# showlab/VideoSwap

Measured on NVIDIA H100. Metric: denoise-steps/sec, 16f 512^2 SD1.5 UNet3D (CFG UNet fwd + CFG combine + DDIM step), higher is better.
Workload: dtype f16

## Files before the change

videoswap_b200/csrc/attention.cu:

```cuda
#include "common.cuh"
#include "kernels.h"

namespace vs {
namespace {

__device__ __forceinline__ void cp_async16(uint32_t dst, const void* src, bool pred) {
  const int sz = pred ? 16 : 0;
  asm volatile("cp.async.cg.shared.global [%0], [%1], 16, %2;" ::"r"(dst), "l"(src), "r"(sz) : "memory");
}
__device__ __forceinline__ void cp_async_commit() { asm volatile("cp.async.commit_group;" ::: "memory"); }
template <int N>
__device__ __forceinline__ void cp_async_wait() {
  asm volatile("cp.async.wait_group %0;" ::"n"(N) : "memory");
}
__device__ __forceinline__ void ldsm_x4(uint32_t addr, uint32_t& r0, uint32_t& r1, uint32_t& r2, uint32_t& r3) {
  asm volatile("ldmatrix.sync.aligned.m8n8.x4.shared.b16 {%0,%1,%2,%3}, [%4];"
               : "=r"(r0), "=r"(r1), "=r"(r2), "=r"(r3)
               : "r"(addr));
}
__device__ __forceinline__ void ldsm_x4_t(uint32_t addr, uint32_t& r0, uint32_t& r1, uint32_t& r2, uint32_t& r3) {
  asm volatile("ldmatrix.sync.aligned.m8n8.x4.trans.shared.b16 {%0,%1,%2,%3}, [%4];"
               : "=r"(r0), "=r"(r1), "=r"(r2), "=r"(r3)
               : "r"(addr));
}
__device__ __forceinline__ void mma16816(float* c, const uint32_t* a, uint32_t b0, uint32_t b1) {
  asm volatile(
      "mma.sync.aligned.m16n8k16.row.col.f32.f16.f16.f32 {%0,%1,%2,%3}, {%4,%5,%6,%7}, {%8,%9}, {%0,%1,%2,%3};"
      : "+f"(c[0]), "+f"(c[1]), "+f"(c[2]), "+f"(c[3])
      : "r"(a[0]), "r"(a[1]), "r"(a[2]), "r"(a[3]), "r"(b0), "r"(b1));
}
__device__ __forceinline__ uint32_t pack_h2(float a, float b) {
  __half2 h = __floats2half2_rn(a, b);
  return *reinterpret_cast<uint32_t*>(&h);
}

template <int DP, int NT>
__device__ __forceinline__ void warp_qk(float (*s)[4], uint32_t q_s, uint32_t k_s, int lds_bytes, int lane) {
#pragma unroll
  for (int n = 0; n < NT; ++n) s[n][0] = s[n][1] = s[n][2] = s[n][3] = 0.f;
#pragma unroll
  for (int kk = 0; kk < DP / 16; ++kk) {
    uint32_t a[4];
    ldsm_x4(q_s + (lane & 15) * lds_bytes + (kk * 16 + (lane >> 4) * 8) * 2, a[0], a[1], a[2], a[3]);
#pragma unroll
    for (int n = 0; n < NT; n += 2) {
      uint32_t b0, b1, b2, b3;
      const int key = n * 8 + (lane & 7) + ((lane >> 4) ? 8 : 0);
// ... 584 lines not shown
```

videoswap_b200/csrc/common.cuh:

```cuda
#pragma once
#include <cuda.h>
#include <cuda_fp16.h>
#include <cuda_runtime.h>
#include <stdint.h>
#include <stdio.h>

namespace vs {

void set_error(const char* fmt, ...);
const char* last_error();

#define VS_CHECK_CUDA(expr)                                                                         \
  do {                                                                                              \
    cudaError_t _e = (expr);                                                                        \
    if (_e != cudaSuccess) {                                                                        \
      vs::set_error("%s:%d CUDA error %s: %s", __FILE__, __LINE__, #expr, cudaGetErrorString(_e)); \
      return 1;                                                                                     \
    }                                                                                               \
  } while (0)

#define VS_REQUIRE(cond, ...)                \
  do {                                       \
    if (!(cond)) {                           \
      vs::set_error(__VA_ARGS__);            \
// ... 100 lines not shown
      ::"r"(dst), "l"(reinterpret_cast<uint64_t>(m)), "r"(bar), "r"(c0), "r"(c1), "r"(c2), "r"(c3)
      : "memory");
}

__device__ __forceinline__ bool elect_one() {
  uint32_t pred;
  asm volatile(
      "{\n\t.reg .pred P;\n\t"
      "elect.sync _|P, 0xffffffff;\n\t"
      "selp.u32 %0, 1, 0, P;\n\t}"
      : "=r"(pred));
  return pred != 0;
}

__device__ __forceinline__ uint32_t cluster_ctarank() {
  uint32_t r;
  asm volatile("mov.u32 %0, %%cluster_ctarank;" : "=r"(r));
  return r;
}
__device__ __forceinline__ void cluster_sync_all() {
  asm volatile("barrier.cluster.arrive.release.aligned;" ::: "memory");
  asm volatile("barrier.cluster.wait.acquire.aligned;" ::: "memory");
}
__device__ __forceinline__ uint32_t mapa_shared(uint32_t addr, uint32_t rank) {
  uint32_t r;
  asm volatile("mapa.shared::cluster.u32 %0, %1, %2;" : "=r"(r) : "r"(addr), "r"(rank));
  return r;
}
__device__ __forceinline__ void named_bar_sync(int id, int nthreads) {
  asm volatile("bar.sync %0, %1;" ::"r"(id), "r"(nthreads) : "memory");
}
__device__ __forceinline__ void named_bar_arrive(int id, int nthreads) {
  asm volatile("bar.arrive %0, %1;" ::"r"(id), "r"(nthreads) : "memory");
}

__device__ __forceinline__ void pdl_trigger() { asm volatile("griddepcontrol.launch_dependents;" ::: "memory"); }
__device__ __forceinline__ void pdl_wait() { asm volatile("griddepcontrol.wait;" ::: "memory"); }

template <int N>
__device__ __forceinline__ void setmaxnreg_dec() { asm volatile("setmaxnreg.dec.sync.aligned.u32 %0;" ::"n"(N)); }
template <int N>
__device__ __forceinline__ void setmaxnreg_inc() { asm volatile("setmaxnreg.inc.sync.aligned.u32 %0;" ::"n"(N)); }

__device__ __forceinline__ void wgmma_fence() { asm volatile("wgmma.fence.sync.aligned;" ::: "memory"); }
__device__ __forceinline__ void wgmma_commit() { asm volatile("wgmma.commit_group.sync.aligned;" ::: "memory"); }
template <int N>
__device__ __forceinline__ void wgmma_wait() { asm volatile("wgmma.wait_group.sync.aligned %0;" ::"n"(N) : "memory"); }

__device__ __forceinline__ uint64_t gmma_desc_sw128(uint32_t smem_addr) {
  uint64_t d = 0;
  d |= (uint64_t)((smem_addr & 0x3FFFF) >> 4);
  d |= (uint64_t)1 << 16;
  d |= (uint64_t)(1024 >> 4) << 32;
  d |= (uint64_t)1 << 62;
  return d;
}
__device__ __forceinline__ uint64_t gmma_desc_sw128_mn(uint32_t smem_addr, uint32_t lbo_bytes) {
  uint64_t d = 0;
  d |= (uint64_t)((smem_addr & 0x3FFFF) >> 4);
  d |= (uint64_t)((lbo_bytes >> 4) & 0x3FFF) << 16;
  d |= (uint64_t)(1024 >> 4) << 32;
  d |= (uint64_t)1 << 62;
  return d;
}

#define VS_R8(i) "+f"(d[i]), "+f"(d[i + 1]), "+f"(d[i + 2]), "+f"(d[i + 3]), "+f"(d[i + 4]), "+f"(d[i + 5]), "+f"(d[i + 6]), "+f"(d[i + 7])
// ... 93 lines not shown
```

videoswap_b200/csrc/gemm.cu:

```cuda
#include <type_traits>

#include "common.cuh"
#include "kernels.h"

namespace vs {

namespace {

constexpr int BM = 128;
constexpr int WG_M = 64;
constexpr int BK = 64;
constexpr int A_STAGE_BYTES = BM * BK * 2;
constexpr uint64_t A_HALF_DESC = (WG_M * BK * 2) >> 4;
constexpr int GEMM_THREADS = 384;
constexpr int SMEM_LIMIT = 227 * 1024;
constexpr int EPI_COLS = 32;
constexpr int EPI_WARP_BYTES = 16 * 64;
constexpr int EPI_BYTES = 8 * EPI_WARP_BYTES;
constexpr int PRODUCER_REGS = 40, CONSUMER_REGS = 232;
enum { EPI_F_GEGLU = 1, EPI_F_RES = 2, EPI_F_RV = 4, EPI_F_LN = 8, EPI_F_LNOUT = 16, EPI_F_QGELU = 32 };

struct GemmParams {
  CUtensorMap tmA, tmA2, tmB;
  int M, N;
  int num_kb;
  int kb_per_tap;
  int kb_src1;
  int taps;
  int a_rank;
  int nimg, H, W, TH, TW, TN, tiles_x, tiles_y;
  int tap_x0, tap_y0, tap_w;
  int osy, osx, ooy, oox, OH, OW;
  int tw_log, thw_log;
  int m_tiles, n_tiles;
  const float* bias;
  const float* rowvec;
  int ldrv;
  int pix_per_batch;
  int rv_mod;
  const float2* ln_stats;
  const float* ln_u;
  const float2* ln_parts;
  int ln_nparts;
  float ln_inv_c;
  float2* ln_sums_out;
  const __half* residual;
  int ldr;
  __half* out;
  int ldc;
  int staged;
  int stages;
};

struct GemmParamsSub : GemmParams {
  CUtensorMap tmS[3];
  int sub_short;
};

struct GemmParamsS2 : GemmParams {
  CUtensorMap tmP[3];
};

template <int BN>
struct Cfg {
  static constexpr bool COOP = BN > 160;
  static constexpr int HALVES = COOP ? 1 : 2;
  static constexpr int B_STAGE_BYTES = BN * BK * 2;
  static constexpr int STAGE_BYTES = A_STAGE_BYTES + B_STAGE_BYTES;
  static constexpr int STAGES_RAW = (SMEM_LIMIT - 2048 - EPI_BYTES) / STAGE_BYTES;
  static constexpr int STAGES = STAGES_RAW > 12 ? 12 : STAGES_RAW;
  static constexpr int SMEM_BYTES = STAGES * STAGE_BYTES + EPI_BYTES + 1024  + 256 ;
  static_assert(B_STAGE_BYTES % 1024 == 0, "B stage must keep 1024-byte alignment for SWIZZLE_128B");
  static_assert(STAGES >= 3, "pipeline too shallow");
  static_assert(BN % 32 == 0 && BN <= 256, "wgmma N");
};

__device__ __forceinline__ uint32_t sw64_off(int row, int chunk) {
  return (uint32_t)(row * 64 + ((chunk ^ ((row >> 1) & 3)) << 4));
}

template <int BN, int EPI, typename Params>
__global__ void __launch_bounds__(GEMM_THREADS, 1) gemm_tc_kernel(const __grid_constant__ Params p) {
  using C = Cfg<BN>;
  constexpr bool SUB = std::is_same<Params, GemmParamsSub>::value;
  constexpr bool S2 = std::is_same<Params, GemmParamsS2>::value;
  constexpr bool GEGLU = (EPI & EPI_F_GEGLU) != 0, HAS_RES = (EPI & EPI_F_RES) != 0, HAS_RV = (EPI & EPI_F_RV) != 0;
  constexpr bool LN = (EPI & EPI_F_LN) != 0;
  constexpr bool LNOUT = (EPI & EPI_F_LNOUT) != 0;
  constexpr bool QGELU = (EPI & EPI_F_QGELU) != 0;
  extern __shared__ uint8_t smem_raw[];
  const uint32_t smem_base = (smem_u32(smem_raw) + 1023u) & ~1023u;
  const uint32_t epi_base = smem_base + C::STAGES * C::STAGE_BYTES;
  const uint32_t bar_base = epi_base + EPI_BYTES;
  auto full_bar = [&](int s) { return bar_base + 8u * s; };
  auto empty_bar = [&](int s) { return bar_base + 8u * (C::STAGES + s); };

  const int warp = threadIdx.x >> 5;
  const int lane = threadIdx.x & 31;
  const int wg = threadIdx.x >> 7;
  const int nst = (p.stages > 0 && p.stages < C::STAGES) ? p.stages : C::STAGES;
  const int total_tiles = p.m_tiles * p.n_tiles;

  if (threadIdx.x == 0) {
    prefetch_tmap(&p.tmA);
    prefetch_tmap(&p.tmB);
    if (p.kb_src1 < p.kb_per_tap) prefetch_tmap(&p.tmA2);
    if constexpr (SUB) {
      if (p.sub_short & 1) prefetch_tmap(&p.tmS[0]);
      if (p.sub_short & 2) prefetch_tmap(&p.tmS[1]);
      if (p.sub_short == 3) prefetch_tmap(&p.tmS[2]);
    }
    if constexpr (S2) {
      for (int k = 0; k < 3; ++k) prefetch_tmap(&p.tmP[k]);
    }
    for (int s = 0; s < C::STAGES; ++s) {
      mbar_init(full_bar(s), 1);
      mbar_init(empty_bar(s), C::COOP ? 8 : 4);
    }
    fence_barrier_init();
  }
  __syncthreads();
  pdl_trigger();
  pdl_wait();

  if (wg == 0) {
    setmaxnreg_dec<PRODUCER_REGS>();
// ... 27 lines not shown
          if constexpr (SUB) {
            const bool sy = short_y && dy == p.tap_y0 + 2, sx = short_x && dx == tap_x0 + 2;
            if (sy || sx) tm = sy ? (sx ? &p.tmS[2] : &p.tmS[0]) : &p.tmS[1];
          }
          int ox = dx, oy = dy;
          if constexpr (S2) {
            const int par = ((dy & 1) << 1) | (dx & 1);
            if (par) tm = &p.tmP[par - 1];
            ox = dx >> 1; oy = dy >> 1;
          }
          const int c = (first ? r : r - kb_src1) * BK;
          mbar_expect_tx(fb, C::STAGE_BYTES);
          if (conv) tma_load_4d(a_dst, tm, fb, c, x0 + ox, y0 + oy, i0);
          else tma_load_2d(a_dst, tm, fb, c, m0);
          tma_load_2d(a_dst + A_STAGE_BYTES, &p.tmB, fb, kcoord, n0);
        }
        __syncwarp();
        kcoord += BK;
        if (++r == kb_per_tap) {
          r = 0;
          if (++dx == tap_x1) { dx = tap_x0; ++dy; }
        }
        if (++pr_s == (uint32_t)nst) { pr_s = 0; pr_ph ^= 1; }
      }
    }
    return;
  }

  setmaxnreg_inc<CONSUMER_REGS>();
  const int g = wg - 1;
  const int wq = warp & 3;
  const int q = lane & 3;
  const int rbase = 16 * wq + (lane >> 2);
  const uint32_t stage_buf = epi_base + (uint32_t)(warp - 4) * EPI_WARP_BYTES;
  const bool has_bias = p.bias != nullptr;
  const bool staged = p.staged != 0;
  const int num_kb = p.num_kb;
  auto tile_pixel = [&](int m_tile, int row) -> int {
    if (p.a_rank == 4) {
      const int x0 = (m_tile % p.tiles_x) * p.TW;
      const int y0 = ((m_tile / p.tiles_x) % p.tiles_y) * p.TH;
      const int i0 = (m_tile / (p.tiles_x * p.tiles_y)) * p.TN;
      const int ti = row >> p.thw_log, rem = row & ((1 << p.thw_log) - 1);
      const int y = y0 + (rem >> p.tw_log), x = x0 + (rem & (p.TW - 1)), img = i0 + ti;
      if constexpr (SUB) {
        const int oy = y * p.osy + p.ooy, ox = x * p.osx + p.oox;
        return ((img < p.nimg) && (y < p.H) && (x < p.W) && (oy < p.OH) && (ox < p.OW)) ? (img * p.OH + oy) * p.OW + ox : -1;
      }
      return ((img < p.nimg) && (y < p.H) && (x < p.W)) ? (img * p.OH + y * p.osy + p.ooy) * p.OW + x * p.osx + p.oox : -1;
    }
    const int px = m_tile * BM + row;
    return px < p.M ? px : -1;
  };

  const int bar_mine = 1 + g, bar_other = 2 - g;
  float acc[C::HALVES][BN / 2];
  uint32_t s = 0, ph = 0;
  for (int t = blockIdx.x, j = 0; t < total_tiles; t += gridDim.x, ++j) {
    const int m_tile = t / p.n_tiles, n_tile = t % p.n_tiles;
    if (!C::COOP && (j & 1) != g) {
      const uint32_t sn = s + (uint32_t)num_kb;
      ph ^= (sn / (uint32_t)nst) & 1u;
      s = sn % (uint32_t)nst;
      continue;
    }
    if (!C::COOP && j > 0) named_bar_sync(bar_mine, 256);
    uint32_t prev = 0;
    for (int kb = 0; kb < num_kb; ++kb) {
      mbar_wait(full_bar(s), ph);
      wgmma_fence();
      const uint32_t a_addr = smem_base + s * C::STAGE_BYTES;
      const uint64_t da = gmma_desc_sw128(a_addr) + (C::COOP ? (uint64_t)g * A_HALF_DESC : 0);
      const uint64_t db = gmma_desc_sw128(a_addr + A_STAGE_BYTES);
#pragma unroll
      for (int k = 0; k < BK / 16; ++k) {
#pragma unroll
        for (int hh = 0; hh < C::HALVES; ++hh)
          wgmma_ss<BN>(acc[hh], da + hh * A_HALF_DESC + 2 * k, db + 2 * k, (kb | k) != 0 ? 1u : 0u);
      }
      wgmma_commit();
      if (kb > 0) {
        wgmma_wait<1>();
        if (lane == 0) mbar_arrive(empty_bar(prev));
      }
      prev = s;
      if (++s == (uint32_t)nst) { s = 0; ph ^= 1; }
    }
    if (!C::COOP && t + (int)gridDim.x < total_tiles) named_bar_arrive(bar_other, 256);
    wgmma_wait<0>();
    if (lane == 0) mbar_arrive(empty_bar(prev));

    const int n0 = n_tile * BN;
#pragma unroll
    for (int hh = 0; hh < C::HALVES; ++hh) {
      const int r0 = WG_M * (C::COOP ? g : hh) + rbase;
      int pix[2];
      pix[0] = tile_pixel(m_tile, r0);
      pix[1] = tile_pixel(m_tile, r0 + 8);
      const float* rv[2] = {nullptr, nullptr};
      if (HAS_RV || !staged) {
#pragma unroll
        for (int h = 0; h < 2; ++h) {
          if (p.rowvec != nullptr && pix[h] >= 0) {
            int ri = pix[h] / p.pix_per_batch;
            if (p.rv_mod > 0) ri %= p.rv_mod;
            rv[h] = p.rowvec + (long long)ri * p.ldrv + n0;
          }
        }
      }
      if (staged) {
        constexpr int OC = GEGLU ? BN / 2 : BN;
        const int oc0 = n_tile * OC;
        const int nsub = (p.N - n0 < BN ? (GEGLU ? (p.N - n0) / 2 : p.N - n0) : OC) / EPI_COLS;
        float la[2] = {1.f, 1.f}, lb[2] = {0.f, 0.f};
        if (LN) {
#pragma unroll
          for (int h = 0; h < 2; ++h) {
            if (pix[h] < 0) continue;
            if (p.ln_nparts > 0) {
              float S = 0.f, Q = 0.f;
              for (int k = 0; k < p.ln_nparts; ++k) {
                const float2 v = __ldg(p.ln_parts + (long long)k * p.M + pix[h]);
                S += v.x; Q += v.y;
              }
              const float mean = S * p.ln_inv_c;
              la[h] = rsqrtf(fmaxf(fmaf(-mean, mean, Q * p.ln_inv_c), 0.f) + 1e-5f);
              lb[h] = -mean * la[h];
            } else {
              const float2 st2 = __ldg(p.ln_stats + pix[h]);
              la[h] = st2.x; lb[h] = st2.y;
            }
          }
        }
        float rs[2] = {0.f, 0.f}, rq[2] = {0.f, 0.f};
        __half* orow[2];
        const __half* rrow[2];
#pragma unroll
        for (int h = 0; h < 2; ++h) {
          const long long px = pix[h] >= 0 ? pix[h] : 0;
          orow[h] = p.out + px * p.ldc + oc0 + q * 8;
          rrow[h] = HAS_RES ? p.residual + px * p.ldr + oc0 + q * 8 : nullptr;
        }
#pragma unroll
        for (int sb = 0; sb < OC / EPI_COLS; ++sb) {
          if (sb >= nsub) break;
          uint4 rr[2];
          if (HAS_RES) {
#pragma unroll
            for (int h = 0; h < 2; ++h) rr[h] = __ldg(reinterpret_cast<const uint4*>(rrow[h] + sb * EPI_COLS));
          }
#pragma unroll
          for (int jj = 0; jj < 4; ++jj) {
            const int j = 4 * sb + jj;
            const int c = 8 * j + 2 * q;
            float2 b = has_bias ? __ldg(reinterpret_cast<const float2*>(p.bias + n0 + c)) : make_float2(0.f, 0.f);
            float2 u = LN ? __ldg(reinterpret_cast<const float2*>(p.ln_u + n0 + c)) : make_float2(0.f, 0.f);
            float2 bg = make_float2(0.f, 0.f), ug = make_float2(0.f, 0.f);
            if (GEGLU) {
              bg = __ldg(reinterpret_cast<const float2*>(p.bias + n0 + BN / 2 + c));
              if (LN) ug = __ldg(reinterpret_cast<const float2*>(p.ln_u + n0 + BN / 2 + c));
            }
#pragma unroll
            for (int h = 0; h < 2; ++h) {
              float f0 = acc[hh][4 * j + 2 * h], f1 = acc[hh][4 * j + 2 * h + 1];
              if (GEGLU) {
                float g0 = acc[hh][4 * (j + BN / 16) + 2 * h], g1 = acc[hh][4 * (j + BN / 16) + 2 * h + 1];
                float bv0 = b.x, bv1 = b.y, bg0 = bg.x, bg1 = bg.y;
                if (LN) {
                  bv0 = fmaf(lb[h], u.x, bv0); bv1 = fmaf(lb[h], u.y, bv1);
                  bg0 = fmaf(lb[h], ug.x, bg0); bg1 = fmaf(lb[h], ug.y, bg1);
                  f0 *= la[h]; f1 *= la[h]; g0 *= la[h]; g1 *= la[h];
                }
                f0 = (f0 + bv0) * gelu_sig(g0 + bg0);
                f1 = (f1 + bv1) * gelu_sig(g1 + bg1);
              } else {
                if (LN) {
                  f0 = fmaf(la[h], f0, fmaf(lb[h], u.x, b.x));
                  f1 = fmaf(la[h], f1, fmaf(lb[h], u.y, b.y));
                } else if (has_bias) {
                  f0 += b.x; f1 += b.y;
                }
                if (HAS_RV && rv[h] != nullptr) {
                  const float2 r2 = __ldg(reinterpret_cast<const float2*>(rv[h] + c));
                  f0 += r2.x; f1 += r2.y;
                }
                if constexpr (QGELU) {
                  f0 = quick_gelu_f(f0); f1 = quick_gelu_f(f1);
                }
              }
              const __half2 hv = __floats2half2_rn(f0, f1);
              asm volatile("st.shared.b32 [%0], %1;" ::"r"(stage_buf + sw64_off((lane >> 2) + 8 * h, jj) + 4 * q),
                           "r"(*reinterpret_cast<const uint32_t*>(&hv)) : "memory");
            }
          }
          __syncwarp();
#pragma unroll
          for (int h = 0; h < 2; ++h) {
            uint4 o;
            asm volatile("ld.shared.v4.b32 {%0,%1,%2,%3}, [%4];" : "=r"(o.x), "=r"(o.y), "=r"(o.z), "=r"(o.w)
                         : "r"(stage_buf + sw64_off((lane >> 2) + 8 * h, q)));
            if (HAS_RES) {
              __half2* oh = reinterpret_cast<__half2*>(&o);
              const __half2* rh = reinterpret_cast<const __half2*>(&rr[h]);
#pragma unroll
              for (int t = 0; t < 4; ++t) oh[t] = __hadd2(oh[t], rh[t]);
            }
            if (pix[h] >= 0) *reinterpret_cast<uint4*>(orow[h] + sb * EPI_COLS) = o;
            if (LNOUT) {
              const __half2* oh = reinterpret_cast<const __half2*>(&o);
              const float2 a = __half22float2(oh[0]), b2 = __half22float2(oh[1]), c2 = __half22float2(oh[2]), d2 = __half22float2(oh[3]);
              rs[h] += ((a.x + a.y) + (b2.x + b2.y)) + ((c2.x + c2.y) + (d2.x + d2.y));
              float q0 = fmaf(a.x, a.x, a.y * a.y), q1 = fmaf(b2.x, b2.x, b2.y * b2.y);
              float q2 = fmaf(c2.x, c2.x, c2.y * c2.y), q3 = fmaf(d2.x, d2.x, d2.y * d2.y);
              rq[h] += (q0 + q1) + (q2 + q3);
            }
          }
          __syncwarp();
        }
        if (LNOUT) {
#pragma unroll
          for (int h = 0; h < 2; ++h) {
            rs[h] += __shfl_xor_sync(0xffffffffu, rs[h], 1); rq[h] += __shfl_xor_sync(0xffffffffu, rq[h], 1);
            rs[h] += __shfl_xor_sync(0xffffffffu, rs[h], 2); rq[h] += __shfl_xor_sync(0xffffffffu, rq[h], 2);
            if (q == 0 && pix[h] >= 0) p.ln_sums_out[(long long)n_tile * p.M + pix[h]] = make_float2(rs[h], rq[h]);
          }
        }
      } else {
#pragma unroll
        for (int j = 0; j < BN / 8; ++j) {
#pragma unroll
          for (int e = 0; e < 4; ++e) {
            const int h = e >> 1, c = 8 * j + 2 * q + (e & 1), n = n0 + c;
            if (n < p.N && pix[h] >= 0) {
              float f = acc[hh][4 * j + e];
              if (has_bias) f += p.bias[n];
              if (rv[h]) f += rv[h][c];
              __half y = __float2half_rn(f);
              if (p.residual) y = __hadd(y, p.residual[(long long)pix[h] * p.ldr + n]);
              p.out[(long long)pix[h] * p.ldc + n] = y;
            }
          }
        }
      }
    }
  }
}

struct ConvTile { int tw, th, tn; };

ConvTile pick_conv_tile(int nimg, int H, int W) {
  ConvTile best{1, 1, BM};
  long long best_cost = -1;
  for (int tw = 1; tw <= BM; tw *= 2) {
    for (int th = 1; tw * th <= BM; th *= 2) {
      const int tn = BM / (tw * th);
      if (tw > 256 || th > 256 || tn > 256) continue;
      const long long cost = (long long)((W + tw - 1) / tw) * tw * ((H + th - 1) / th) * th * ((nimg + tn - 1) / tn) * tn;
      if (best_cost < 0 || cost < best_cost || (cost == best_cost && tw > best.tw)) {
        best_cost = cost;
        best = ConvTile{tw, th, tn};
      }
    }
  }
  return best;
}

template <int BN, int EPI, typename Params = GemmParams>
int launch(cudaStream_t st, const Params& p) {
  using C = Cfg<BN>;
  static bool configured = false;
  if (!configured) {
    VS_CHECK_CUDA(cudaFuncSetAttribute(gemm_tc_kernel<BN, EPI, Params>, cudaFuncAttributeMaxDynamicSharedMemorySize, C::SMEM_BYTES));
    configured = true;
  }
  const int total = p.m_tiles * p.n_tiles;
  int ctas = num_sms();
  const int cap = get_option("gemm_ctas");
  if (cap > 0 && cap < ctas) ctas = cap;
  return launch_pdl(gemm_tc_kernel<BN, EPI, Params>, dim3(total < ctas ? total : ctas), dim3(GEMM_THREADS), C::SMEM_BYTES, st, 1, p);
}

template <int BN>
int launch_linear(cudaStream_t st, const GemmParams& p) {
  const int epi = (p.residual ? EPI_F_RES : 0) | (p.rowvec ? EPI_F_RV : 0) | ((p.ln_stats || p.ln_parts) ? EPI_F_LN : 0) |
                  (p.ln_sums_out ? EPI_F_LNOUT : 0);
  switch (epi) {
    case EPI_F_LNOUT: return launch<BN, EPI_F_LNOUT>(st, p);
    case EPI_F_LNOUT | EPI_F_RES: return launch<BN, EPI_F_LNOUT | EPI_F_RES>(st, p);
    case EPI_F_LN: return launch<BN, EPI_F_LN>(st, p);
    case EPI_F_LN | EPI_F_RV: return launch<BN, EPI_F_LN | EPI_F_RV>(st, p);
    case 0: return launch<BN, 0>(st, p);
    case EPI_F_RES: return launch<BN, EPI_F_RES>(st, p);
    case EPI_F_RV: return launch<BN, EPI_F_RV>(st, p);
    case EPI_F_RES | EPI_F_RV: return launch<BN, EPI_F_RES | EPI_F_RV>(st, p);
    default: set_error("gemm_tc: unsupported epilogue combination 0x%x", epi); return 2;
  }
}

int pick_bn(int m_tiles, int N, int num_kb) {
  if (N <= 64) return 64;
  int best = 128;
  long long best_cost = -1;
// ... 110 lines not shown
        const bool used = k == 2 ? ps.sub_short == 3 : ((ps.sub_short >> k) & 1) != 0;
        if (used && make_tmap_f16(&ps.tmS[k], a.A - shift[k], 4, dims, str, box, 1)) return 3;
      }
    }
    if (two) {
      const uint64_t dims[4] = {(uint64_t)a.K2, (uint64_t)a.W, (uint64_t)a.H, (uint64_t)a.nimg};
      const uint64_t str[3] = {(uint64_t)a.lda2 * 2, (uint64_t)a.lda2 * 2 * a.W, (uint64_t)a.lda2 * 2 * a.W * a.H};
      if (make_tmap_f16(&p.tmA2, a.A2, 4, dims, str, box, 1)) return 3;
    }
  } else {
    p.a_rank = 2;
    p.m_tiles = (a.M + BM - 1) / BM;
    const uint32_t box[2] = {BK, BM};
    {
      const uint64_t dims[2] = {(uint64_t)a.K1, (uint64_t)a.M};
      const uint64_t str[1] = {(uint64_t)a.lda1 * 2};
      if (make_tmap_f16(&p.tmA, a.A, 2, dims, str, box, 1)) return 3;
    }
    if (two) {
      const uint64_t dims[2] = {(uint64_t)a.K2, (uint64_t)a.M};
      const uint64_t str[1] = {(uint64_t)a.lda2 * 2};
      if (make_tmap_f16(&p.tmA2, a.A2, 2, dims, str, box, 1)) return 3;
    }
  }

  int bn = a.force_bn;
  if (a.mode == EPI_GEGLU) {
    bn = 2 * kGegluGranule;
    VS_REQUIRE(a.N % bn == 0, "gemm_tc: GEGLU needs N %% %d == 0 (N=%d)", bn, a.N);
    VS_REQUIRE(a.bias != nullptr && a.residual == nullptr && a.rowvec == nullptr, "gemm_tc: GEGLU takes a bias only");
  } else if (bn == 0) {
    bn = pick_bn(p.m_tiles, a.N, p.num_kb);
  }
  VS_REQUIRE(bn == 64 || bn == 128 || bn == 160 || bn == 256, "gemm_tc: unsupported BLOCK_N %d", bn);
  p.n_tiles = (a.N + bn - 1) / bn;
  {
    const uint64_t dims[2] = {(uint64_t)Ktot, (uint64_t)a.N};
    const uint64_t str[1] = {(uint64_t)Ktot * 2};
    const uint32_t box[2] = {BK, (uint32_t)bn};
    if (make_tmap_f16(&p.tmB, a.Bw, 2, dims, str, box, 1)) return 3;
  }
  const int out_cols = (a.mode == EPI_GEGLU) ? a.N / 2 : a.N;
  p.staged = (out_cols % EPI_COLS == 0) && (a.ldc % 8 == 0) && ((reinterpret_cast<uintptr_t>(a.out) & 15) == 0) &&
             (!a.residual || ((a.ldr % 8 == 0) && ((reinterpret_cast<uintptr_t>(a.residual) & 15) == 0))) &&
             (!a.bias || (reinterpret_cast<uintptr_t>(a.bias) & 15) == 0) &&
             (!a.rowvec || ((reinterpret_cast<uintptr_t>(a.rowvec) & 15) == 0 && p.ldrv % 4 == 0));
  if (a.mode == EPI_QUICK_GELU)
    VS_REQUIRE(a.taps == 1 && p.staged && a.residual == nullptr && a.rowvec == nullptr && !a.ln_stats && !a.ln_parts &&
               a.ln_sums_out == nullptr && (bn == 128 || bn == 256),
               "gemm_tc: the quick-GELU epilogue takes a plain GEMM with a bias only, N %% 32 == 0 and BLOCK_N 128 / 256 (got %d)", bn);
  if (!p.staged) VS_REQUIRE(a.mode == EPI_LINEAR, "gemm_tc: GEGLU output needs 32-column aligned, 16-byte strided rows");
  if (a.ln_stats || a.ln_parts) VS_REQUIRE(p.staged && (reinterpret_cast<uintptr_t>(a.ln_u) & 15) == 0, "gemm_tc: folded LayerNorm needs the staged epilogue");
  if (a.ln_sums_out) VS_REQUIRE(p.staged, "gemm_tc: row statistics output needs the staged epilogue (N %% 32 == 0, aligned rows)");
  ProfScope prof(st, a.taps != 1 ? PC_CONV : PC_GEMM, 2.0 * a.M * (double)a.N * Ktot, 1, a.M, a.N, Ktot);
  if (a.mode == EPI_GEGLU) {
    if (p.ln_stats || p.ln_parts) return launch<256, EPI_F_GEGLU | EPI_F_LN>(st, p);
    return launch<256, EPI_F_GEGLU>(st, p);
  }
  if (a.mode == EPI_QUICK_GELU) return bn == 256 ? launch<256, EPI_F_QGELU>(st, p) : launch<128, EPI_F_QGELU>(st, p);
  if (s2) {
    VS_REQUIRE(a.residual == nullptr && a.rowvec == nullptr && a.ln_sums_out == nullptr && p.staged,
               "gemm_tc: the stride-2 conv takes a bias only and needs N %% 32 == 0");
    static_cast<GemmParams&>(p2) = p;
    switch (bn) {
      case 64: return launch<64, 0, GemmParamsS2>(st, p2);
      case 128: return launch<128, 0, GemmParamsS2>(st, p2);
      case 256: return launch<256, 0, GemmParamsS2>(st, p2);
      default: return launch<160, 0, GemmParamsS2>(st, p2);
    }
  }
  if (sub && ((OH | OW) & 1)) {
    VS_REQUIRE(a.residual == nullptr && a.rowvec == nullptr && p.staged, "gemm_tc: an odd-sized sub-pixel conv takes a bias only");
    switch (bn) {
      case 64: return launch<64, 0, GemmParamsSub>(st, ps);
      case 128: return launch<128, 0, GemmParamsSub>(st, ps);
      case 256: return launch<256, 0, GemmParamsSub>(st, ps);
      default: return launch<160, 0, GemmParamsSub>(st, ps);
    }
  }
  switch (bn) {
    case 64: return launch_linear<64>(st, p);
    case 128: return launch_linear<128>(st, p);
    case 256: return launch_linear<256>(st, p);
    default: return launch_linear<160>(st, p);
  }
// ... 29 lines not shown
```

Baseline: 10.94.

## Prefetch GEMM epilogue operands into shared memory with cp.async during mainloop

Before each tile's K-loop, the consumer warpgroups now issue cp.async copies of the bias, LayerNorm u vector, per-batch row vectors and the first residual chunks into a new double-buffered shared-memory operand area. Per-row LayerNorm statistics are computed or preloaded before the mainloop as well. The aim is to hide global-memory latency in the epilogue behind the wgmma work. In exchange, shared memory per epilogue variant grows, which can reduce the number of pipeline stages, and a fallback path handles row-vector spans that are too large for the buffer.

```diff
diff --git a/videoswap_b200/csrc/attention.cu b/videoswap_b200/csrc/attention.cu
--- a/videoswap_b200/csrc/attention.cu
+++ b/videoswap_b200/csrc/attention.cu
@@ -4,15 +4,6 @@
 namespace vs {
 namespace {
 
-__device__ __forceinline__ void cp_async16(uint32_t dst, const void* src, bool pred) {
-  const int sz = pred ? 16 : 0;
-  asm volatile("cp.async.cg.shared.global [%0], [%1], 16, %2;" ::"r"(dst), "l"(src), "r"(sz) : "memory");
-}
-__device__ __forceinline__ void cp_async_commit() { asm volatile("cp.async.commit_group;" ::: "memory"); }
-template <int N>
-__device__ __forceinline__ void cp_async_wait() {
-  asm volatile("cp.async.wait_group %0;" ::"n"(N) : "memory");
-}
 __device__ __forceinline__ void ldsm_x4(uint32_t addr, uint32_t& r0, uint32_t& r1, uint32_t& r2, uint32_t& r3) {
   asm volatile("ldmatrix.sync.aligned.m8n8.x4.shared.b16 {%0,%1,%2,%3}, [%4];"
                : "=r"(r0), "=r"(r1), "=r"(r2), "=r"(r3)
diff --git a/videoswap_b200/csrc/common.cuh b/videoswap_b200/csrc/common.cuh
--- a/videoswap_b200/csrc/common.cuh
+++ b/videoswap_b200/csrc/common.cuh
@@ -156,6 +156,16 @@
 }
 __device__ __forceinline__ void named_bar_arrive(int id, int nthreads) {
   asm volatile("bar.arrive %0, %1;" ::"r"(id), "r"(nthreads) : "memory");
+}
+
+__device__ __forceinline__ void cp_async16(uint32_t dst, const void* src, bool pred) {
+  const int sz = pred ? 16 : 0;
+  asm volatile("cp.async.cg.shared.global [%0], [%1], 16, %2;" ::"r"(dst), "l"(src), "r"(sz) : "memory");
+}
+__device__ __forceinline__ void cp_async_commit() { asm volatile("cp.async.commit_group;" ::: "memory"); }
+template <int N>
+__device__ __forceinline__ void cp_async_wait() {
+  asm volatile("cp.async.wait_group %0;" ::"n"(N) : "memory");
 }
 
 __device__ __forceinline__ void pdl_trigger() { asm volatile("griddepcontrol.launch_dependents;" ::: "memory"); }
diff --git a/videoswap_b200/csrc/gemm.cu b/videoswap_b200/csrc/gemm.cu
--- a/videoswap_b200/csrc/gemm.cu
+++ b/videoswap_b200/csrc/gemm.cu
@@ -38,6 +38,7 @@
   int ldrv;
   int pix_per_batch;
   int rv_mod;
+  int rv_slots;
   const float2* ln_stats;
   const float* ln_u;
   const float2* ln_parts;
@@ -61,15 +62,22 @@
   CUtensorMap tmP[3];
 };
 
-template <int BN>
+constexpr int rv_rows(int bn) { return bn > 160 ? 9 : 16; }
+
+template <int BN, int EPI>
 struct Cfg {
   static constexpr bool COOP = BN > 160;
   static constexpr int HALVES = COOP ? 1 : 2;
   static constexpr int B_STAGE_BYTES = BN * BK * 2;
   static constexpr int STAGE_BYTES = A_STAGE_BYTES + B_STAGE_BYTES;
-  static constexpr int STAGES_RAW = (SMEM_LIMIT - 2048 - EPI_BYTES) / STAGE_BYTES;
+  static constexpr int VEC_BYTES = BN * 4 * ((EPI & EPI_F_LN) ? 2 : 1);
+  static constexpr int RV_BYTES = (EPI & EPI_F_RV) ? rv_rows(BN) * BN * 4 : 0;
+  static constexpr int RES_SLOTS = (EPI & EPI_F_RES) ? (COOP ? 2 : BN / EPI_COLS) : 0;
+  static constexpr int RES_BYTES = RES_SLOTS * WG_M * EPI_COLS * 2;
+  static constexpr int OPS_BYTES = VEC_BYTES + RV_BYTES + RES_BYTES;
+  static constexpr int STAGES_RAW = (SMEM_LIMIT - 2048 - EPI_BYTES - 2 * OPS_BYTES) / STAGE_BYTES;
   static constexpr int STAGES = STAGES_RAW > 12 ? 12 : STAGES_RAW;
-  static constexpr int SMEM_BYTES = STAGES * STAGE_BYTES + EPI_BYTES + 1024  + 256 ;
+  static constexpr int SMEM_BYTES = STAGES * STAGE_BYTES + EPI_BYTES + 2 * OPS_BYTES + 1024  + 256 ;
   static_assert(B_STAGE_BYTES % 1024 == 0, "B stage must keep 1024-byte alignment for SWIZZLE_128B");
   static_assert(STAGES >= 3, "pipeline too shallow");
   static_assert(BN % 32 == 0 && BN <= 256, "wgmma N");
@@ -81,7 +89,7 @@
 
 template <int BN, int EPI, typename Params>
 __global__ void __launch_bounds__(GEMM_THREADS, 1) gemm_tc_kernel(const __grid_constant__ Params p) {
-  using C = Cfg<BN>;
+  using C = Cfg<BN, EPI>;
   constexpr bool SUB = std::is_same<Params, GemmParamsSub>::value;
   constexpr bool S2 = std::is_same<Params, GemmParamsS2>::value;
   constexpr bool GEGLU = (EPI & EPI_F_GEGLU) != 0, HAS_RES = (EPI & EPI_F_RES) != 0, HAS_RV = (EPI & EPI_F_RV) != 0;
@@ -91,7 +99,8 @@
   extern __shared__ uint8_t smem_raw[];
   const uint32_t smem_base = (smem_u32(smem_raw) + 1023u) & ~1023u;
   const uint32_t epi_base = smem_base + C::STAGES * C::STAGE_BYTES;
-  const uint32_t bar_base = epi_base + EPI_BYTES;
+  const uint32_t ops_base = epi_base + EPI_BYTES;
+  const uint32_t bar_base = ops_base + 2 * C::OPS_BYTES;
   auto full_bar = [&](int s) { return bar_base + 8u * s; };
   auto empty_bar = [&](int s) { return bar_base + 8u * (C::STAGES + s); };
 
@@ -185,10 +194,21 @@
   const int wq = warp & 3;
   const int q = lane & 3;
   const int rbase = 16 * wq + (lane >> 2);
+  const int ct = threadIdx.x & 127;
   const uint32_t stage_buf = epi_base + (uint32_t)(warp - 4) * EPI_WARP_BYTES;
+  const uint32_t vec_buf = ops_base + (uint32_t)g * C::OPS_BYTES;
+  const uint32_t rv_buf = vec_buf + C::VEC_BYTES;
+  const uint32_t res_buf = rv_buf + C::RV_BYTES;
+  const float* vec_s = reinterpret_cast<const float*>(smem_raw + (vec_buf - smem_u32(smem_raw)));
+  const float* rv_s = vec_s + C::VEC_BYTES / 4;
+  const uint4* res_s = reinterpret_cast<const uint4*>(rv_s + C::RV_BYTES / 4);
+  const int bar_ops = 3 + g;
   const bool has_bias = p.bias != nullptr;
   const bool staged = p.staged != 0;
   const int num_kb = p.num_kb;
+  const long long npix = p.a_rank == 4 ? (long long)p.nimg * p.OH * p.OW : p.M;
+  constexpr int OC = GEGLU ? BN / 2 : BN;
+  constexpr int NSUB = OC / EPI_COLS;
   auto tile_pixel = [&](int m_tile, int row) -> int {
     if (p.a_rank == 4) {
       const int x0 = (m_tile % p.tiles_x) * p.TW;
@@ -205,6 +225,12 @@
     const int px = m_tile * BM + row;
     return px < p.M ? px : -1;
   };
+  auto res_copy = [&](const int* px, int oc0, int sb, int slot) {
+#pragma unroll
+    for (int h = 0; h < 2; ++h)
+      cp_async16(res_buf + (uint32_t)(((slot * WG_M + rbase + 8 * h) * 4 + q) * 16),
+                 p.residual + (long long)(px[h] >= 0 ? px[h] : 0) * p.ldr + oc0 + sb * EPI_COLS + q * 8, px[h] >= 0);
+  };
 
   const int bar_mine = 1 + g, bar_other = 2 - g;
   float acc[C::HALVES][BN / 2];
@@ -217,7 +243,81 @@
       s = sn % (uint32_t)nst;
       continue;
     }
+    const int n0 = n_tile * BN;
+    const int oc0 = n_tile * OC;
+    const int nsub = (p.N - n0 < BN ? (GEGLU ? (p.N - n0) / 2 : p.N - n0) : OC) / EPI_COLS;
+    int pix[C::HALVES][2];
+    float la[C::HALVES][2], lb[C::HALVES][2];
+#pragma unroll
+    for (int hh = 0; hh < C::HALVES; ++hh) {
+      const int r0 = WG_M * (C::COOP ? g : hh) + rbase;
+      pix[hh][0] = tile_pixel(m_tile, r0);
+      pix[hh][1] = tile_pixel(m_tile, r0 + 8);
+#pragma unroll
+      for (int h = 0; h < 2; ++h) { la[hh][h] = 1.f; lb[hh][h] = 0.f; }
+    }
+    int rv0 = 0;
+    constexpr bool LN_REGS = LN && C::COOP;
+    constexpr int LN_REG = 8;
+    float2 lnv[LN_REGS ? 2 : 1][LN_REGS ? LN_REG : 1];
+    const bool ln_late = LN_REGS && p.ln_nparts <= LN_REG;
+    if (ln_late) {
+#pragma unroll
+      for (int h = 0; h < 2; ++h) {
+        const int px = pix[0][h];
+#pragma unroll
+        for (int k = 0; k < (LN_REGS ? LN_REG : 1); ++k) {
+          const bool in = px >= 0 && (p.ln_nparts > 0 ? k < p.ln_nparts : k == 0);
+          lnv[h][k] = in ? __ldg(p.ln_nparts > 0 ? p.ln_parts + (long long)k * p.M + px : p.ln_stats + px) : make_float2(0.f, 0.f);
+        }
+      }
+    } else if (LN) {
+#pragma unroll
+      for (int hh = 0; hh < C::HALVES; ++hh) {
+#pragma unroll
+        for (int h = 0; h < 2; ++h) {
+          const int px = pix[hh][h];
+          if (px < 0) continue;
+          if (p.ln_nparts > 0) {
+            float S = 0.f, Q = 0.f;
+            for (int k = 0; k < p.ln_nparts; ++k) {
+              const float2 v = __ldg(p.ln_parts + (long long)k * p.M + px);
+              S += v.x; Q += v.y;
+            }
+            const float mean = S * p.ln_inv_c;
+            la[hh][h] = rsqrtf(fmaxf(fmaf(-mean, mean, Q * p.ln_inv_c), 0.f) + 1e-5f);
+            lb[hh][h] = -mean * la[hh][h];
+          } else {
+            const float2 st2 = __ldg(p.ln_stats + px);
+            la[hh][h] = st2.x; lb[hh][h] = st2.y;
+          }
+        }
+      }
+    }
+    if (HAS_RES && staged) {
+      for (int sb = 0; sb < C::RES_SLOTS && sb < nsub; ++sb) res_copy(pix[0], oc0, sb, sb);
+      cp_async_commit();
+    }
     if (!C::COOP && j > 0) named_bar_sync(bar_mine, 256);
+    if (staged) {
+      if (C::COOP && j > 0) named_bar_sync(bar_ops, 128);
+      for (int i = ct; i < BN / 4; i += 128) {
+        const bool in = n0 + 4 * i < p.N;
+        if (has_bias) cp_async16(vec_buf + 16 * i, p.bias + (in ? n0 + 4 * i : 0), in);
+        if (LN) cp_async16(vec_buf + 4 * BN + 16 * i, p.ln_u + (in ? n0 + 4 * i : 0), in);
+      }
+      if (HAS_RV) {
+        rv0 = tile_pixel(m_tile, 0) / p.pix_per_batch;
+        for (int i = ct; i < p.rv_slots * (BN / 4); i += 128) {
+          const int sl = i / (BN / 4), c = 4 * (i % (BN / 4));
+          const int ri = rv0 + sl;
+          const bool in = (long long)ri * p.pix_per_batch < npix && n0 + c < p.N;
+          const long long row = p.rv_mod > 0 ? ri % p.rv_mod : ri;
+          cp_async16(rv_buf + 4 * (sl * BN + c), p.rowvec + (in ? row * p.ldrv + n0 + c : 0), in);
+        }
+      }
+      cp_async_commit();
+    }
     uint32_t prev = 0;
     for (int kb = 0; kb < num_kb; ++kb) {
       mbar_wait(full_bar(s), ph);
@@ -242,155 +342,155 @@
     if (!C::COOP && t + (int)gridDim.x < total_tiles) named_bar_arrive(bar_other, 256);
     wgmma_wait<0>();
     if (lane == 0) mbar_arrive(empty_bar(prev));
-
-    const int n0 = n_tile * BN;
+    if (ln_late) {
+#pragma unroll
+      for (int h = 0; h < 2; ++h) {
+        if (pix[0][h] < 0) continue;
+        if (p.ln_nparts > 0) {
+          float S = 0.f, Q = 0.f;
+#pragma unroll
+          for (int k = 0; k < (LN_REGS ? LN_REG : 1); ++k) {
+            if (k < p.ln_nparts) { S += lnv[h][k].x; Q += lnv[h][k].y; }
+          }
+          const float mean = S * p.ln_inv_c;
+          la[0][h] = rsqrtf(fmaxf(fmaf(-mean, mean, Q * p.ln_inv_c), 0.f) + 1e-5f);
+          lb[0][h] = -mean * la[0][h];
+        } else {
+          la[0][h] = lnv[h][0].x; lb[0][h] = lnv[h][0].y;
+        }
+      }
+    }
+
+    if (staged) {
+      cp_async_wait<0>();
+      named_bar_sync(bar_ops, 128);
+    }
 #pragma unroll
     for (int hh = 0; hh < C::HALVES; ++hh) {
-      const int r0 = WG_M * (C::COOP ? g : hh) + rbase;
-      int pix[2];
-      pix[0] = tile_pixel(m_tile, r0);
-      pix[1] = tile_pixel(m_tile, r0 + 8);
-      const float* rv[2] = {nullptr, nullptr};
-      if (HAS_RV || !staged) {
-#pragma unroll
-        for (int h = 0; h < 2; ++h) {
-          if (p.rowvec != nullptr && pix[h] >= 0) {
-            int ri = pix[h] / p.pix_per_batch;
-            if (p.rv_mod > 0) ri %= p.rv_mod;
-            rv[h] = p.rowvec + (long long)ri * p.ldrv + n0;
-          }
-        }
-      }
       if (staged) {
-        constexpr int OC = GEGLU ? BN / 2 : BN;
-        const int oc0 = n_tile * OC;
-        const int nsub = (p.N - n0 < BN ? (GEGLU ? (p.N - n0) / 2 : p.N - n0) : OC) / EPI_COLS;
-        float la[2] = {1.f, 1.f}, lb[2] = {0.f, 0.f};
-        if (LN) {
-#pragma unroll
-          for (int h = 0; h < 2; ++h) {
-            if (pix[h] < 0) continue;
-            if (p.ln_nparts > 0) {
-              float S = 0.f, Q = 0.f;
-              for (int k = 0; k < p.ln_nparts; ++k) {
-                const float2 v = __ldg(p.ln_parts + (long long)k * p.M + pix[h]);
-                S += v.x; Q += v.y;
-              }
-              const float mean = S * p.ln_inv_c;
-              la[h] = rsqrtf(fmaxf(fmaf(-mean, mean, Q * p.ln_inv_c), 0.f) + 1e-5f);
-              lb[h] = -mean * la[h];
-            } else {
-              const float2 st2 = __ldg(p.ln_stats + pix[h]);
-              la[h] = st2.x; lb[h] = st2.y;
-            }
-          }
-        }
         float rs[2] = {0.f, 0.f}, rq[2] = {0.f, 0.f};
         __half* orow[2];
-        const __half* rrow[2];
+        const float* rvr[2] = {rv_s, rv_s};
 #pragma unroll
         for (int h = 0; h < 2; ++h) {
-          const long long px = pix[h] >= 0 ? pix[h] : 0;
+          const long long px = pix[hh][h] >= 0 ? pix[hh][h] : 0;
           orow[h] = p.out + px * p.ldc + oc0 + q * 8;
-          rrow[h] = HAS_RES ? p.residual + px * p.ldr + oc0 + q * 8 : nullptr;
-        }
-#pragma unroll
-        for (int sb = 0; sb < OC / EPI_COLS; ++sb) {
-          if (sb >= nsub) break;
-          uint4 rr[2];
-          if (HAS_RES) {
-#pragma unroll
-            for (int h = 0; h < 2; ++h) rr[h] = __ldg(reinterpret_cast<const uint4*>(rrow[h] + sb * EPI_COLS));
-          }
-#pragma unroll
-          for (int jj = 0; jj < 4; ++jj) {
-            const int j = 4 * sb + jj;
-            const int c = 8 * j + 2 * q;
-            float2 b = has_bias ? __ldg(reinterpret_cast<const float2*>(p.bias + n0 + c)) : make_float2(0.f, 0.f);
-            float2 u = LN ? __ldg(reinterpret_cast<const float2*>(p.ln_u + n0 + c)) : make_float2(0.f, 0.f);
-            float2 bg = make_float2(0.f, 0.f), ug = make_float2(0.f, 0.f);
-            if (GEGLU) {
-              bg = __ldg(reinterpret_cast<const float2*>(p.bias + n0 + BN / 2 + c));
-              if (LN) ug = __ldg(reinterpret_cast<const float2*>(p.ln_u + n0 + BN / 2 + c));
+          if (HAS_RV && pix[hh][h] >= 0) rvr[h] = rv_s + ((int)(px / p.pix_per_batch) - rv0) % p.rv_slots * BN;
+        }
+#pragma unroll
+        for (int sb = 0; sb < NSUB; ++sb) {
+          const int u = NSUB * hh + sb;
+          if (sb < nsub) {
+            if constexpr (HAS_RES) {
+              if (u >= C::RES_SLOTS) cp_async_wait<C::RES_SLOTS - 1>();
             }
 #pragma unroll
+            for (int jj = 0; jj < 4; ++jj) {
+              const int j = 4 * sb + jj;
+              const int c = 8 * j + 2 * q;
+              float2 b = has_bias ? *reinterpret_cast<const float2*>(vec_s + c) : make_float2(0.f, 0.f);
+              float2 u = LN ? *reinterpret_cast<const float2*>(vec_s + BN + c) : make_float2(0.f, 0.f);
+              float2 bg = make_float2(0.f, 0.f), ug = make_float2(0.f, 0.f);
+              if (GEGLU) {
+                bg = *reinterpret_cast<const float2*>(vec_s + BN / 2 + c);
+                if (LN) ug = *reinterpret_cast<const float2*>(vec_s + BN + BN / 2 + c);
+              }
+#pragma unroll
+              for (int h = 0; h < 2; ++h) {
+                float f0 = acc[hh][4 * j + 2 * h], f1 = acc[hh][4 * j + 2 * h + 1];
+                if (GEGLU) {
+                  float g0 = acc[hh][4 * (j + BN / 16) + 2 * h], g1 = acc[hh][4 * (j + BN / 16) + 2 * h + 1];
+                  float bv0 = b.x, bv1 = b.y, bg0 = bg.x, bg1 = bg.y;
+                  if (LN) {
+                    bv0 = fmaf(lb[hh][h], u.x, bv0); bv1 = fmaf(lb[hh][h], u.y, bv1);
+                    bg0 = fmaf(lb[hh][h], ug.x, bg0); bg1 = fmaf(lb[hh][h], ug.y, bg1);
+                    f0 *= la[hh][h]; f1 *= la[hh][h]; g0 *= la[hh][h]; g1 *= la[hh][h];
+                  }
+                  f0 = (f0 + bv0) * gelu_sig(g0 + bg0);
+                  f1 = (f1 + bv1) * gelu_sig(g1 + bg1);
+                } else {
+                  if (LN) {
+                    f0 = fmaf(la[hh][h], f0, fmaf(lb[hh][h], u.x, b.x));
+                    f1 = fmaf(la[hh][h], f1, fmaf(lb[hh][h], u.y, b.y));
+                  } else if (has_bias) {
+                    f0 += b.x; f1 += b.y;
+                  }
+                  if (HAS_RV && pix[hh][h] >= 0) {
+                    const float2 r2 = *reinterpret_cast<const float2*>(rvr[h] + c);
+                    f0 += r2.x; f1 += r2.y;
+                  }
+                  if constexpr (QGELU) {
+                    f0 = quick_gelu_f(f0); f1 = quick_gelu_f(f1);
+                  }
+                }
+                const __half2 hv = __floats2half2_rn(f0, f1);
+                asm volatile("st.shared.b32 [%0], %1;" ::"r"(stage_buf + sw64_off((lane >> 2) + 8 * h, jj) + 4 * q),
+                             "r"(*reinterpret_cast<const uint32_t*>(&hv)) : "memory");
+              }
+            }
+            __syncwarp();
+#pragma unroll
             for (int h = 0; h < 2; ++h) {
-              float f0 = acc[hh][4 * j + 2 * h], f1 = acc[hh][4 * j + 2 * h + 1];
-              if (GEGLU) {
-                float g0 = acc[hh][4 * (j + BN / 16) + 2 * h], g1 = acc[hh][4 * (j + BN / 16) + 2 * h + 1];
-                float bv0 = b.x, bv1 = b.y, bg0 = bg.x, bg1 = bg.y;
-                if (LN) {
-                  bv0 = fmaf(lb[h], u.x, bv0); bv1 = fmaf(lb[h], u.y, bv1);
-                  bg0 = fmaf(lb[h], ug.x, bg0); bg1 = fmaf(lb[h], ug.y, bg1);
-                  f0 *= la[h]; f1 *= la[h]; g0 *= la[h]; g1 *= la[h];
-                }
-                f0 = (f0 + bv0) * gelu_sig(g0 + bg0);
-                f1 = (f1 + bv1) * gelu_sig(g1 + bg1);
-              } else {
-                if (LN) {
-                  f0 = fmaf(la[h], f0, fmaf(lb[h], u.x, b.x));
-                  f1 = fmaf(la[h], f1, fmaf(lb[h], u.y, b.y));
-                } else if (has_bias) {
-                  f0 += b.x; f1 += b.y;
-                }
-                if (HAS_RV && rv[h] != nullptr) {
-                  const float2 r2 = __ldg(reinterpret_cast<const float2*>(rv[h] + c));
-                  f0 += r2.x; f1 += r2.y;
-                }
-                if constexpr (QGELU) {
-                  f0 = quick_gelu_f(f0); f1 = quick_gelu_f(f1);
-                }
+              uint4 o;
+              asm volatile("ld.shared.v4.b32 {%0,%1,%2,%3}, [%4];" : "=r"(o.x), "=r"(o.y), "=r"(o.z), "=r"(o.w)
+                           : "r"(stage_buf + sw64_off((lane >> 2) + 8 * h, q)));
+              if constexpr (HAS_RES) {
+                const uint4 rr = res_s[(u % C::RES_SLOTS * WG_M + rbase + 8 * h) * 4 + q];
+                __half2* oh = reinterpret_cast<__half2*>(&o);
+                const __half2* rh = reinterpret_cast<const __half2*>(&rr);
+#pragma unroll
+                for (int t = 0; t < 4; ++t) oh[t] = __hadd2(oh[t], rh[t]);
               }
-              const __half2 hv = __floats2half2_rn(f0, f1);
-              asm volatile("st.shared.b32 [%0], %1;" ::"r"(stage_buf + sw64_off((lane >> 2) + 8 * h, jj) + 4 * q),
-                           "r"(*reinterpret_cast<const uint32_t*>(&hv)) : "memory");
+              if (pix[hh][h] >= 0) *reinterpret_cast<uint4*>(orow[h] + sb * EPI_COLS) = o;
+              if (LNOUT) {
+                const __half2* oh = reinterpret_cast<const __half2*>(&o);
+                const float2 a = __half22float2(oh[0]), b2 = __half22float2(oh[1]), c2 = __half22float2(oh[2]), d2 = __half22float2(oh[3]);
+                rs[h] += ((a.x + a.y) + (b2.x + b2.y)) + ((c2.x + c2.y) + (d2.x + d2.y));
+                float q0 = fmaf(a.x, a.x, a.y * a.y), q1 = fmaf(b2.x, b2.x, b2.y * b2.y);
+                float q2 = fmaf(c2.x, c2.x, c2.y * c2.y), q3 = fmaf(d2.x, d2.x, d2.y * d2.y);
+                rq[h] += (q0 + q1) + (q2 + q3);
+              }
             }
-          }
-          __syncwarp();
-#pragma unroll
-          for (int h = 0; h < 2; ++h) {
-            uint4 o;
-            asm volatile("ld.shared.v4.b32 {%0,%1,%2,%3}, [%4];" : "=r"(o.x), "=r"(o.y), "=r"(o.z), "=r"(o.w)
-                         : "r"(stage_buf + sw64_off((lane >> 2) + 8 * h, q)));
-            if (HAS_RES) {
-              __half2* oh = reinterpret_cast<__half2*>(&o);
-              const __half2* rh = reinterpret_cast<const __half2*>(&rr[h]);
-#pragma unroll
-              for (int t = 0; t < 4; ++t) oh[t] = __hadd2(oh[t], rh[t]);
-            }
-            if (pix[h] >= 0) *reinterpret_cast<uint4*>(orow[h] + sb * EPI_COLS) = o;
-            if (LNOUT) {
-              const __half2* oh = reinterpret_cast<const __half2*>(&o);
-              const float2 a = __half22float2(oh[0]), b2 = __half22float2(oh[1]), c2 = __half22float2(oh[2]), d2 = __half22float2(oh[3]);
-              rs[h] += ((a.x + a.y) + (b2.x + b2.y)) + ((c2.x + c2.y) + (d2.x + d2.y));
-              float q0 = fmaf(a.x, a.x, a.y * a.y), q1 = fmaf(b2.x, b2.x, b2.y * b2.y);
-              float q2 = fmaf(c2.x, c2.x, c2.y * c2.y), q3 = fmaf(d2.x, d2.x, d2.y * d2.y);
-              rq[h] += (q0 + q1) + (q2 + q3);
-            }
-          }
-          __syncwarp();
+            __syncwarp();
+          }
+          if constexpr (HAS_RES) {
+            const int u2 = u + C::RES_SLOTS, h2 = u2 / NSUB, sb2 = u2 % NSUB;
+            if (u2 < C::HALVES * NSUB && sb2 < nsub) res_copy(pix[h2 < C::HALVES ? h2 : 0], oc0, sb2, u2 % C::RES_SLOTS);
+            cp_async_commit();
+          }
         }
         if (LNOUT) {
 #pragma unroll
           for (int h = 0; h < 2; ++h) {
             rs[h] += __shfl_xor_sync(0xffffffffu, rs[h], 1); rq[h] += __shfl_xor_sync(0xffffffffu, rq[h], 1);
             rs[h] += __shfl_xor_sync(0xffffffffu, rs[h], 2); rq[h] += __shfl_xor_sync(0xffffffffu, rq[h], 2);
-            if (q == 0 && pix[h] >= 0) p.ln_sums_out[(long long)n_tile * p.M + pix[h]] = make_float2(rs[h], rq[h]);
+            if (q == 0 && pix[hh][h] >= 0) p.ln_sums_out[(long long)n_tile * p.M + pix[hh][h]] = make_float2(rs[h], rq[h]);
           }
         }
       } else {
+        const int* px = pix[hh];
+        const float* rv[2] = {nullptr, nullptr};
+#pragma unroll
+        for (int h = 0; h < 2; ++h) {
+          if (p.rowvec != nullptr && px[h] >= 0) {
+            int ri = px[h] / p.pix_per_batch;
+            if (p.rv_mod > 0) ri %= p.rv_mod;
+            rv[h] = p.rowvec + (long long)ri * p.ldrv + n0;
+          }
+        }
 #pragma unroll
         for (int j = 0; j < BN / 8; ++j) {
 #pragma unroll
           for (int e = 0; e < 4; ++e) {
             const int h = e >> 1, c = 8 * j + 2 * q + (e & 1), n = n0 + c;
-            if (n < p.N && pix[h] >= 0) {
+            if (n < p.N && px[h] >= 0) {
               float f = acc[hh][4 * j + e];
-              if (has_bias) f += p.bias[n];
+              if (LN) f = fmaf(la[hh][h], f, fmaf(lb[hh][h], p.ln_u[n], p.bias[n]));
+              else if (has_bias) f += p.bias[n];
               if (rv[h]) f += rv[h][c];
               __half y = __float2half_rn(f);
-              if (p.residual) y = __hadd(y, p.residual[(long long)pix[h] * p.ldr + n]);
-              p.out[(long long)pix[h] * p.ldc + n] = y;
+              if (p.residual) y = __hadd(y, p.residual[(long long)px[h] * p.ldr + n]);
+              p.out[(long long)px[h] * p.ldc + n] = y;
             }
           }
         }
@@ -420,7 +520,7 @@
 
 template <int BN, int EPI, typename Params = GemmParams>
 int launch(cudaStream_t st, const Params& p) {
-  using C = Cfg<BN>;
+  using C = Cfg<BN, EPI>;
   static bool configured = false;
   if (!configured) {
     VS_CHECK_CUDA(cudaFuncSetAttribute(gemm_tc_kernel<BN, EPI, Params>, cudaFuncAttributeMaxDynamicSharedMemorySize, C::SMEM_BYTES));
@@ -597,6 +697,13 @@
   } else if (bn == 0) {
     bn = pick_bn(p.m_tiles, a.N, p.num_kb);
   }
+  long long rv_need = 0;
+  if (a.rowvec) {
+    const long long span = a.taps != 1 ? (long long)p.TN * p.OH * p.OW : BM;
+    rv_need = (span - 1) / p.pix_per_batch + 2;
+    if (p.rv_mod > 0 && p.rv_mod < rv_need) rv_need = p.rv_mod;
+    p.rv_slots = (int)(rv_need < rv_rows(bn) ? rv_need : rv_rows(bn));
+  }
   VS_REQUIRE(bn == 64 || bn == 128 || bn == 160 || bn == 256, "gemm_tc: unsupported BLOCK_N %d", bn);
   p.n_tiles = (a.N + bn - 1) / bn;
   {
@@ -609,13 +716,14 @@
   p.staged = (out_cols % EPI_COLS == 0) && (a.ldc % 8 == 0) && ((reinterpret_cast<uintptr_t>(a.out) & 15) == 0) &&
              (!a.residual || ((a.ldr % 8 == 0) && ((reinterpret_cast<uintptr_t>(a.residual) & 15) == 0))) &&
              (!a.bias || (reinterpret_cast<uintptr_t>(a.bias) & 15) == 0) &&
-             (!a.rowvec || ((reinterpret_cast<uintptr_t>(a.rowvec) & 15) == 0 && p.ldrv % 4 == 0));
+             (!a.rowvec || ((reinterpret_cast<uintptr_t>(a.rowvec) & 15) == 0 && p.ldrv % 4 == 0 && rv_need <= rv_rows(bn)));
   if (a.mode == EPI_QUICK_GELU)
     VS_REQUIRE(a.taps == 1 && p.staged && a.residual == nullptr && a.rowvec == nullptr && !a.ln_stats && !a.ln_parts &&
                a.ln_sums_out == nullptr && (bn == 128 || bn == 256),
                "gemm_tc: the quick-GELU epilogue takes a plain GEMM with a bias only, N %% 32 == 0 and BLOCK_N 128 / 256 (got %d)", bn);
   if (!p.staged) VS_REQUIRE(a.mode == EPI_LINEAR, "gemm_tc: GEGLU output needs 32-column aligned, 16-byte strided rows");
-  if (a.ln_stats || a.ln_parts) VS_REQUIRE(p.staged && (reinterpret_cast<uintptr_t>(a.ln_u) & 15) == 0, "gemm_tc: folded LayerNorm needs the staged epilogue");
+  if (a.ln_stats || a.ln_parts) VS_REQUIRE((p.staged || rv_need > rv_rows(bn)) && (reinterpret_cast<uintptr_t>(a.ln_u) & 15) == 0,
+                                           "gemm_tc: folded LayerNorm needs the staged epilogue");
   if (a.ln_sums_out) VS_REQUIRE(p.staged, "gemm_tc: row statistics output needs the staged epilogue (N %% 32 == 0, aligned rows)");
   ProfScope prof(st, a.taps != 1 ? PC_CONV : PC_GEMM, 2.0 * a.M * (double)a.N * Ktot, 1, a.M, a.N, Ktot);
   if (a.mode == EPI_GEGLU) {
```

Measured after the change: 11.23, median of 6. +2.7%, better.
